# at-cg/PHI

Measured on AMD Instinct MI355X. Metric: read Gbases/s scored (49-hap MHC graph stand-in synMHC-49); reads resident in HBM, parsing and H2D excluded, higher is better.
Workload: dtype u64

## Files before the change

### phi_amd/build.py

```python
import os
import subprocess
import sys

ROOT = os.path.dirname(os.path.dirname(os.path.abspath(__file__)))
CSRC = os.path.join(ROOT, "phi_amd", "csrc")
HIPCC = os.environ.get("HIPCC", "/opt/rocm/bin/hipcc")
ARCH = "gfx950"

HIP_SOURCES = ["sketch.hip", "sketch_pooled.hip", "table.hip", "anchors.hip", "contexts.hip", "dp.hip", "dp_events.hip", "phi_abi.hip", "phi_solve.hip", "solve_dev.hip", "phi_comm.hip", "phi_ipc.hip", "reads_text.hip", "walk_text.hip", "edit.hip", "edit_path.hip", "inflate.hip", "gfa_text.hip"]
HIP_HEADERS = ["phi_dev.h", "phi_kernels.h", "phi_ctx.h", "sketch.hip", "sketch_phases.inc", "sketch_minima.inc", "sketch_rounds.inc", "edit_band.inc", os.path.join("..", "..", "include", "phi_amd.h")]


def _run(cmd, cwd=None):
    print("+", " ".join(cmd), flush=True)
    subprocess.check_call(cmd, cwd=cwd)


def _stale(target, deps):
    if not os.path.exists(target):
        return True
    t = os.path.getmtime(target)
    return any(os.path.getmtime(d) > t for d in deps if os.path.exists(d))


EXTRA_FLAGS = {"sketch_pooled.hip": ["-mllvm", "-disable-machine-licm"]}


def build_device(force=False):
    objdir = os.path.join(ROOT, "build", "obj")
    os.makedirs(objdir, exist_ok=True)
    hdrs = [os.path.join(CSRC, h) for h in HIP_HEADERS]
    objs = []
    for src in HIP_SOURCES:
        s = os.path.join(CSRC, src)
        o = os.path.join(objdir, src.replace(".hip", ".o"))
        if force or _stale(o, [s] + hdrs):
            _run([HIPCC, f"--offload-arch={ARCH}", "-O3", "-std=c++17", "-fPIC", "-Wall", "-Wno-unused-function"]
                 + EXTRA_FLAGS.get(src, []) + ["-c", s, "-o", o])
        objs.append(o)
    lib = os.path.join(ROOT, "phi_amd", "libphi_amd.so")
    if force or _stale(lib, objs):
        tmp = f"{lib}.{os.getpid()}.tmp"
        _run([HIPCC, f"--offload-arch={ARCH}", "-shared", "-fPIC", "-o", tmp] + objs + ["-ldl"])
        os.replace(tmp, lib)
    return lib


def build_host(force=False):
    hostdir = os.path.join(CSRC, "host")
    if not os.path.isdir(hostdir):
        return None
    _run(["make", "-C", hostdir] + (["-B"] if force else []))
    return os.path.join(ROOT, "phi_amd", "libphi_host.so")


def build_all(force=False):
    build_device(force)
    build_host(force)


if __name__ == "__main__":
    build_all(force="--force" in sys.argv)
```

### phi_amd/csrc/sketch.hip

```cpp
#include <hip/hip_runtime.h>
#include <type_traits>
#include <hip/hip_ext.h>
#include "phi_dev.h"
#include "phi_kernels.h"
#ifndef PHI_ABL
#define PHI_ABL 0
#endif

#define TPB PHI_TPB
#define Q 8

int64_t phi_sketch_num_blocks(int64_t n_bases);


static __device__ __forceinline__ void pack_ascii_word(int64_t wi, const uint8_t *__restrict__ bases, int64_t n,
                                                       uint64_t *__restrict__ words, int64_t n_words,
                                                       uint32_t *__restrict__ badbits,
                                                       unsigned long long *__restrict__ n_bad)
{
    if (wi >= n_words + 4) return;
    if (wi >= n_words) {
        if (wi < n_words + 2) words[wi] = 0;
        if (badbits) badbits[wi] = 0;
        return;
// ... 275 lines not shown
            else {
                const KRef prev = window_best_bytes(A.ascii, a - 1, k, w);
                emit = !(prev.pos == best.pos && prev.rc == best.rc) && khash_bytes<LONGK>(A.ascii, prev, k) != h;
            }
        }
        const unsigned long long bal = __ballot(emit);
        bool novel = false;
        if (emit) {
            const int rank = n_emit + __popcll(bal & ((1ull << lane) - 1));
            if (MODE == PHI_MODE_WRITE) {
                A.out_hash[out_base + rank] = h;
                A.out_pos[out_base + rank] = pos;
            } else if (MODE == PHI_MODE_PROBE) {
                novel = probe_table(A, h);
            }
        }
        if (MODE == PHI_MODE_PROBE) {
            const OverflowArgs O{A.ov_list, A.ov_count, A.ov_cap, A.err};
            n_nov += overflow_novel(O, novel, h, lane);
        }
        n_emit += __popcll(bal);
    }
    (void)chunk;
}


#define WCH PHI_WCH
#define SWW 32
#define SBW 16
#define SM(l) s_mp[(l) + ((l) >> 3)]

__host__ __device__ static inline int phi_wave_mp_u64(int w)
{
    const int M = WCH + w, P = (M + 63) / 64;
    const int slots = ((M - 1) / P + 1) * P;
    return ((slots + 8) * 9) / 8 + 8;
}
__host__ __device__ static inline int phi_wave_items(int w, int k) { return 1 + WCH + WCH / (w + k + 1) + 2; }
__host__ __device__ static inline int phi_wave_region_u64(int w, int k, bool pos)
{
    const int item_bytes = pos ? 4 : 2;
    return phi_wave_mp_u64(w) + SWW + 2 * SBW + ((phi_wave_items(w, k) + 4) * item_bytes + 7) / 8
#if PHI_ABL == 4
           + 256
#endif
        ;
}

__device__ __forceinline__ uint64_t min_u62(uint64_t a, uint64_t b)
{
    double r;
    asm("v_min_f64 %0, %1, %2" : "=v"(r) : "v"(__longlong_as_double((long long)a)), "v"(__longlong_as_double((long long)b)));
    return (uint64_t)__double_as_longlong(r);
}

__device__ __forceinline__ uint64_t wave_prev_u64(uint64_t v, uint64_t first, int lane)
{
    const uint32_t lo = (uint32_t)__builtin_amdgcn_update_dpp(0, (int)(uint32_t)v, 0x138, 0xF, 0xF, false);
    const uint32_t hi = (uint32_t)__builtin_amdgcn_update_dpp(0, (int)(uint32_t)(v >> 32), 0x138, 0xF, 0xF, false);
    const uint64_t p = ((uint64_t)hi << 32) | lo;
    return lane == 0 ? first : p;
}

__device__ __forceinline__ int wave_scan_inclusive(int v)
{
    v += __builtin_amdgcn_update_dpp(0, v, 0x111, 0xF, 0xF, true);
    v += __builtin_amdgcn_update_dpp(0, v, 0x112, 0xF, 0xF, true);
    v += __builtin_amdgcn_update_dpp(0, v, 0x114, 0xF, 0xF, true);
    v += __builtin_amdgcn_update_dpp(0, v, 0x118, 0xF, 0xF, true);
    v += __builtin_amdgcn_update_dpp(0, v, 0x142, 0xA, 0xF, false);
    v += __builtin_amdgcn_update_dpp(0, v, 0x143, 0xC, 0xF, false);
    return v;
}

template <int MODE>
static __device__ __forceinline__ void bytes_role(const PhiSketchArgs &A, const unsigned long long *batch_bad,
                                                  int64_t blk, int64_t n_blk, unsigned long long *s_all)
{
    const int lane = threadIdx.x & 63, wid = threadIdx.x >> 6;
    if (!A.allslow && batch_bad && *batch_bad == 0) return;
    const int64_t N = A.n_bases;
    const int64_t n_chunks = (N + WCH - 1) / WCH;
    const int64_t n_sw = N / 64 + 2;
    unsigned long long *s_bits = s_all + (size_t)wid * 2 * SBW, *s_bad = s_bits + SBW;
    for (int64_t chunk = blk * (TPB / 64) + wid; chunk < n_chunks; chunk += n_blk * (TPB / 64)) {
        const int64_t c0 = chunk * WCH;
        unsigned long long my_bad = 0;
        wave_sync();
        if (lane < SBW) {
            const int64_t wi = (c0 >> 6) - 1 + lane;
            s_bits[lane] = (wi >= 0 && wi < n_sw) ? A.starts[wi] : 0;
        } else if (lane < 2 * SBW) {
            const int64_t wi = (c0 >> 6) - 1 + (lane - SBW);
            if (A.badbits) my_bad = (wi >= 0 && wi < n_sw) ? A.badbits[wi] : 0;
            s_bad[lane - SBW] = my_bad;
        }
        const bool chunk_bad = __ballot(my_bad != 0) != 0ull;
        wave_sync();
        int n_emit = 0, n_nov = 0;
        if (A.allslow || chunk_bad) {
            const int64_t out_base = (MODE == PHI_MODE_WRITE) ? A.block_off[chunk] : 0;
            if (A.k > PHI_MAX_K_PACKED) slow_windows<MODE, true>(A, c0, chunk, lane, A.k, A.w, s_bits, s_bad, A.allslow != 0, out_base, n_emit, n_nov);
            else slow_windows<MODE>(A, c0, chunk, lane, A.k, A.w, s_bits, s_bad, A.allslow != 0, out_base, n_emit, n_nov);
        }
        if (MODE == PHI_MODE_COUNT) {
            if (lane == 0) A.block_cnt[chunk] = n_emit;
        }
    }
}



template <class AT>
__device__ __forceinline__ void clean_finish(const AT &A, int64_t gw, int64_t n_waves, int lane)
{
    if (gw == 0 && lane == 0 && A.ov_zero) *A.ov_zero = 0;
    if (A.ipc_mb && A.ipc_need) {
        while (__hip_atomic_load(A.ipc_mb + PHI_MB_GATHERED, __ATOMIC_RELAXED, __HIP_MEMORY_SCOPE_AGENT) < A.ipc_need) __builtin_amdgcn_s_sleep(32);
    }
    if (gw * 64 < A.q_n_hit_words)
        for (int64_t i = gw * 64 + lane; i < A.q_n_hit_words; i += n_waves * 64) A.q_hit_words[i] = 0;
    if (gw * 64 < A.q_n_stripe_words)
        for (int64_t i = gw * 64 + lane; i < A.q_n_stripe_words; i += n_waves * 64) A.q_stripes[i] = 0;
}

struct StartProbe { int64_t base; int64_t v; int64_t nx; };
__device__ __forceinline__ StartProbe start_probe_issue(const PhiSketchArgs &A, int64_t c0, int lane)
{
    const int64_t lo_b = c0 - 64 > 0 ? c0 - 64 : 0;
    int64_t g = (int64_t)(((unsigned long long)lo_b * A.reads_per_base_q32) >> 32) - 24;
    g = g < 0 ? 0 : (g > A.n_reads - 63 ? (A.n_reads - 63 > 0 ? A.n_reads - 63 : 0) : g);
    StartProbe p;
    p.base = g;
    const int64_t idx = g + lane;
    p.v = idx <= A.n_reads ? A.read_off[idx] : INT64_MAX;
    p.nx = idx + 1 <= A.n_reads ? A.read_off[idx + 1] : INT64_MAX;
    return p;
}
__device__ __forceinline__ void set_start_bit(unsigned long long *s_bits, int64_t p, int64_t lo_b)
{
    const int bit = (int)(p - lo_b);
    atomicOr(reinterpret_cast<unsigned int *>(s_bits) + (bit >> 5), 1u << (bit & 31));
}
__device__ __forceinline__ void start_bits_from_offsets(const PhiSketchArgs &A, int64_t c0, int lane, StartProbe pr,
                                                        unsigned long long *s_bits)
{
    const int64_t lo_b = c0 - 64, hi_b = lo_b + 64 * SBW;
    const unsigned long long ge = __ballot(pr.v >= lo_b), lt = __ballot(pr.v < hi_b);
    if ((pr.base == 0 || !(ge & 1ull)) && !(lt >> 63)) {
        if (pr.base + lane < A.n_reads && pr.v >= lo_b && pr.v < hi_b && pr.nx > pr.v) set_start_bit(s_bits, pr.v, lo_b);
        return;
    }
    {
        int64_t vm = __shfl(pr.v, 32, 64);
        if (vm == INT64_MAX) vm = A.n_bases;
        int64_t nb_all = A.n_bases, nr_all = A.n_reads;
        asm volatile("" : "+s"(nb_all), "+s"(nr_all));
        const double mean = (double)nb_all / (double)nr_all;
        int64_t g = pr.base + 32 + (int64_t)((double)(lo_b - vm) / mean) - 24;
        g = g < 0 ? 0 : (g > A.n_reads - 63 ? (A.n_reads - 63 > 0 ? A.n_reads - 63 : 0) : g);
        const int64_t idx = g + lane;
        const int64_t v2 = idx <= A.n_reads ? A.read_off[idx] : INT64_MAX;
        const int64_t nx2 = idx + 1 <= A.n_reads ? A.read_off[idx + 1] : INT64_MAX;
        const unsigned long long ge2 = __ballot(v2 >= lo_b), lt2 = __ballot(v2 < hi_b);
        if ((g == 0 || !(ge2 & 1ull)) && !(lt2 >> 63)) {
            if (idx < A.n_reads && v2 >= lo_b && v2 < hi_b && nx2 > v2) set_start_bit(s_bits, v2, lo_b);
            return;
        }
    }
    int64_t lo = 0, hi = A.n_reads;
    int64_t base = pr.base, stride = 1, v = pr.v;
    for (int round = 0; round < 64 && lo < hi; round++) {
        if (round) {
            stride = (hi - lo + 63) / 64;
            base = lo;
            const int64_t idx = base + lane * stride;
            v = idx <= A.n_reads ? A.read_off[idx] : INT64_MAX;
        }
        const unsigned long long g2 = __ballot(v >= lo_b);
        const int f = g2 ? __ffsll((long long)g2) - 1 : 64;
        if (f == 0) { hi = base < hi ? base : hi; }
        else {
            const int64_t below = base + (int64_t)(f - 1) * stride;
            lo = below + 1 > lo ? below + 1 : lo;
            if (f < 64) { const int64_t at = base + (int64_t)f * stride; hi = at < hi ? at : hi; }
        }
    }
    for (int64_t r = lo + lane;; r += 64) {
        int64_t p = INT64_MAX, nx = INT64_MAX;
        if (r < A.n_reads) { p = A.read_off[r]; nx = A.read_off[r + 1]; }
        if (p >= lo_b && p < hi_b && nx > p) set_start_bit(s_bits, p, lo_b);
        if (__shfl(p, 63, 64) >= hi_b) break;
    }
}

__device__ __forceinline__ void start_bits_uniform(const PhiSketchArgs &A, int64_t c0, int lane, unsigned long long *s_bits)
{
    const int64_t org = c0 - 64, hi_b = org + 64 * SBW;
    const int64_t from = org > 0 ? org : 0;
    const uint32_t L = (uint32_t)A.uniform_len;
    if (A.n_bases <= 0xFFFFFFFFll) {
        const uint32_t x = (uint32_t)__builtin_amdgcn_readfirstlane((int)(uint32_t)from);
        uint32_t q = __umulhi(x, A.inv_len_q32);
        uint32_t r = x - q * L;
        if (r >= L) { q++; r -= L; }
        const uint32_t first = x + (r ? L - r : 0u);
        const uint64_t p = (uint64_t)first + (uint64_t)(uint32_t)lane * (uint64_t)L;
        if (first >= x && (int64_t)p < hi_b && (int64_t)p < A.n_bases) set_start_bit(s_bits, (int64_t)p, org);
        return;
    }
    int64_t q = (int64_t)((double)from * A.inv_len);
    int64_t r = from - q * (int64_t)L;
    if (r < 0) { q--; r += L; }
    if (r >= (int64_t)L) { q++; r -= L; }
    const int64_t p = (q + (r != 0) + lane) * (int64_t)L;
    if (p < hi_b && p < A.n_bases) set_start_bit(s_bits, p, org);
}

template <int ONE = 0>
__device__ __forceinline__ uint4 load_bases16(const uint8_t *__restrict__ ascii, int64_t N, int64_t c0, int lane)
{
    const int64_t b = c0 - 32 + 16 * (int64_t)lane;
    if (b >= 0 && b + 16 <= N && (((uintptr_t)ascii + (uintptr_t)b) & 15) == 0) return *reinterpret_cast<const uint4 *>(ascii + b);
    uint32_t x[4] = {0x41414141u, 0x41414141u, 0x41414141u, 0x41414141u};
    if (b + 16 > 0 && b < N) {
#pragma unroll
        for (int j = 0; j < 16; j++)
            if (b + j >= 0 && b + j < N) x[j >> 2] = (x[j >> 2] & ~(0xFFu << (8 * (j & 3)))) | ((uint32_t)ascii[b + j] << (8 * (j & 3)));
    }
    return make_uint4(x[0], x[1], x[2], x[3]);
}

#ifndef PHI_SKETCH_POOLED_TU
template <int MODE, bool WIDE, int KT, int WT>
__global__ void __launch_bounds__(TPB, MODE == PHI_MODE_PROBE ? 6 : 1) phi_sketch_kernel(PhiSketchArgs A)
{
    constexpr bool FUSED = MODE == PHI_MODE_PROBE;
    constexpr bool NEED_POS = MODE == PHI_MODE_WRITE;
    constexpr bool FMIN = !NEED_POS && KT > 0 && KT <= 31;
    extern __shared__ uint64_t s_dyn[];

    const int lane = threadIdx.x & 63, wid = threadIdx.x >> 6;
    const int k = KT > 0 ? KT : A.k, w = WT ? WT : A.w;
    const int64_t N = A.n_bases;
    const int64_t chunk = (int64_t)blockIdx.x * (TPB / 64) + wid;
    const int64_t c0 = chunk * WCH;
    if (FUSED && A.ipc_mb && chunk == 0 && lane == 0)
        __hip_atomic_store(A.ipc_mb + PHI_MB_SCORED, A.ipc_scored, __ATOMIC_RELEASE, __HIP_MEMORY_SCOPE_AGENT);
    if (c0 >= N) {
        if (FUSED && A.q_clean) clean_finish(A, chunk, (int64_t)gridDim.x * (TPB / 64), lane);
        return;
    }
    const uint64_t kmask = phi_kmask(k);
    const int M = WCH + w;
    const int span = w + k - 1;
    const bool have_bad = FUSED || A.badbits != nullptr;

    using MetaT = typename std::conditional<NEED_POS, uint32_t, uint16_t>::type;
    constexpr uint32_t ITEM_FIRST = NEED_POS ? 1u << 31 : 1u << 15;
    constexpr uint32_t ITEM_NOEMIT = NEED_POS ? 1u << 30 : 1u << 14;
    uint64_t *s_mp = s_dyn + (size_t)wid * phi_wave_region_u64(w, k, NEED_POS);
    uint64_t *s_words = s_mp + phi_wave_mp_u64(w);
    unsigned long long *s_bits = (unsigned long long *)(s_words + SWW);
    unsigned long long *s_bad = s_bits + SBW;
    MetaT *s_meta = (MetaT *)(s_bad + SBW);
    uint64_t *s_q = s_mp + lane * (Q + 1);

    constexpr bool POOL = false;
    bool chunk_bad = false;
    int ncand = 0, n_emit = 0, n_log = 0, n_nov_slow = 0;
    int64_t out_base = 0;
    uint4 xn = make_uint4(0, 0, 0, 0);
    const int ci = 0, mine = 1;
    const int64_t stride = 0;
#include "sketch_phases.inc"

#if PHI_ABL == 15
    { asm volatile("" :: "v"(ncand)); return; }
#endif
#if PHI_ABL == 2
    ncand = 0;
#endif
#include "sketch_rounds.inc"

    if (FUSED && chunk_bad) {
        int n_emit_slow = 0;
        slow_windows<MODE>(A, c0, chunk, lane, k, w, s_bits, s_bad, false, 0, n_emit_slow, n_nov_slow);
        n_emit += n_emit_slow;
    }
    if (FUSED && A.q_clean) clean_finish(A, chunk, (int64_t)gridDim.x * (TPB / 64), lane);
    if (MODE == PHI_MODE_COUNT) {
        if (lane == 0) A.block_cnt[chunk] = n_emit;
    } else if (MODE == PHI_MODE_PROBE) {
        if (lane == 0) {
            const int cap = 1 << A.nov_shift;
            A.nov_cnt[A.log_base + chunk] = (uint16_t)(n_log < cap ? n_log : cap);
            const int n_nov_wave = n_log + n_nov_slow;
            const int stripe = (int)(chunk & (PHI_STRIPES - 1)) * 8;
            if (n_nov_wave && A.n_logged) atomicAdd(A.n_logged + stripe, (unsigned long long)n_nov_wave);
            if (n_emit && A.n_emitted) atomicAdd(A.n_emitted + stripe, (unsigned long long)n_emit);
        }
    }
}

__host__ __device__ static inline int phi_win_items_u64(int w, int k) { return ((phi_wave_items(w, k) + 4) * 2 + 7) / 8; }
__host__ __device__ static inline int phi_win_mp_u64(int R, int s, int w, int k)
{
    const int kmers = 9 * R * s;
    const int minima = 9 * (64 + 1) + phi_win_items_u64(w, k);
    return kmers > minima ? kmers : minima;
}
__host__ __device__ static inline int phi_win_region_u64(int R, int s, int w, int k) { return phi_win_mp_u64(R, s, w, k); }

__device__ __forceinline__ void stage_bad_bits(const uint8_t *__restrict__ ascii, int64_t N, int64_t c0, int lane,
                                               unsigned long long *s_bad)
{
    uint32_t bad = 0;
    if (lane < 62) {
        const uint4 v = load_bases16<1>(ascii, N, c0, lane);
        const uint32_t x[4] = {v.x, v.y, v.z, v.w};
#pragma unroll
        for (int b = 0; b < 16; b++) bad |= (uint32_t)(!phi_is_acgt((x[b >> 2] >> (8 * (b & 3))) & 0xFFu)) << b;
    }
    reinterpret_cast<uint16_t *>(s_bad)[lane < 62 ? lane + 2 : lane - 62] = (uint16_t)bad;
}

__device__ __forceinline__ void slow_windows_reads(const PhiSketchArgs &A, int64_t r0, int nr, int L, int V, int64_t c0, int lane,
                                                   int k, int w, const unsigned long long *s_bad, int &n_emit, int &n_nov)
{
    const int span = w + k - 1, n_win = nr * V;
    for (int q0 = 0; q0 < n_win; q0 += 64) {
        const int q = q0 + lane;
        const int rl = q / V, v = q - rl * V;
        const int64_t a = (r0 + rl) * (int64_t)L + v;
        const int lp = (int)(a - (c0 - 64));
        const bool todo = q < n_win && range_has_bit(s_bad, lp - 1, lp + span - 1);
        bool emit = false;
        uint64_t h = 0;
        if (todo) {
            const KRef best = window_best_bytes(A.ascii, a, k, w);
            h = khash_bytes<false>(A.ascii, best, k);
            if (v == 0) emit = h != PHI_EMPTY_KEY;
            else {
                const KRef prev = window_best_bytes(A.ascii, a - 1, k, w);
                emit = !(prev.pos == best.pos && prev.rc == best.rc) && khash_bytes<false>(A.ascii, prev, k) != h;
            }
        }
        const unsigned long long bal = __ballot(emit);
        const bool novel = emit && probe_table(A, h);
        const OverflowArgs O{A.ov_list, A.ov_count, A.ov_cap, A.err};
        n_nov += overflow_novel(O, novel, h, lane);
        n_emit += __popcll(bal);
    }
}

template <bool WIDE, int KT, int WT>
__global__ void __launch_bounds__(TPB, 7) phi_sketch_win_kernel(PhiSketchArgs A)
{
    constexpr int MODE = PHI_MODE_PROBE;
    constexpr bool NEED_POS = false;
    constexpr bool FMIN = KT > 0 && KT <= 31;
    static_assert(KT >= 0, "k <= 32");
    extern __shared__ uint64_t s_dyn[];

    const int lane = threadIdx.x & 63, wid = threadIdx.x >> 6;
    const int k = KT > 0 ? KT : A.k, w = WT ? WT : A.w;
    const int64_t N = A.n_bases;
    const int L = A.uniform_len, span = w + k - 1, V = L - span + 1;
    const int G = (V + Q - 1) / Q, s = G + (w + Q - 1) / Q, R = A.win_reads;
    const int64_t chunk = (int64_t)blockIdx.x * (TPB / 64) + wid;
    const int64_t rd0 = chunk * R;
    if (A.ipc_mb && chunk == 0 && lane == 0)
        __hip_atomic_store(A.ipc_mb + PHI_MB_SCORED, A.ipc_scored, __ATOMIC_RELEASE, __HIP_MEMORY_SCOPE_AGENT);
    if (rd0 >= A.n_reads) {
        if (A.q_clean) clean_finish(A, chunk, (int64_t)gridDim.x * (TPB / 64), lane);
        return;
    }
    const int nr = A.n_reads - rd0 < R ? (int)(A.n_reads - rd0) : R;
    const uint64_t kmask = phi_kmask(k);
    const int64_t c0 = (rd0 * (int64_t)L) & ~(int64_t)31;
    const int rl = (int)(((float)lane + 0.5f) * (1.0f / (float)G)), j = lane - rl * G;
    const bool live = rl < nr;

    using MetaT = uint16_t;
    constexpr uint32_t ITEM_FIRST = 1u << 15;
    constexpr uint32_t ITEM_NOEMIT = 1u << 14;
    uint64_t *s_mp = s_dyn + (size_t)wid * phi_win_region_u64(R, s, w, k);
    uint64_t *s_words = s_mp;
    unsigned long long *s_bad = (unsigned long long *)s_mp;
    MetaT *s_meta = (MetaT *)(s_mp + 9 * (64 + 1));
    uint64_t *s_q = s_mp + (live ? 9 * (rl * s + j) : 0);

    bool chunk_bad;
    {
        const uint4 v = load_bases16<1>(A.ascii, N, c0, lane);
        const uint32_t x[4] = {v.x, v.y, v.z, v.w};
        uint32_t code = 0, bad = 0;
#pragma unroll
        for (int q = 0; q < 4; q++) {
            const uint32_t t = ((x[q] >> 1) ^ (x[q] >> 2)) & 0x03030303u;
            const uint32_t c8 = (t * 0x40100401u) >> 24;
            code = (code << 8) | c8;
            if (__builtin_amdgcn_perm(0x54474341u, 0x54474341u, t) != (x[q] & 0xDFDFDFDFu)) {
#pragma unroll
                for (int b = 0; b < 4; b++) bad |= (uint32_t)(!phi_is_acgt((x[q] >> (8 * b)) & 0xFFu)) << (4 * q + b);
            }
        }
        reinterpret_cast<uint32_t *>(s_words)[lane ^ 1] = code;
        chunk_bad = __ballot(lane < 62 && bad != 0) != 0ull;
    }
    wave_sync();

    {
        int n = 0, u = 0;
        uint64_t F = 0, Rc = 0, nxt = 0;
        if (live) {
            const int n_km = L - k + 1, P = (n_km + G - 1) / G;
            const int t0 = j * P;
            n = n_km - t0 < P ? n_km - t0 : P;
            if (n > 0) {
                const int lb = (int)((rd0 + rl) * (int64_t)L + t0 - c0) + 32;
                F = lds_extract64(s_words, lb) >> (64 - 2 * k);
                nxt = lds_extract64(s_words, lb + k);
                u = 8 * s * rl + 1 + t0;
            }
        }
        wave_sync();
        if (n > 0) {
            Rc = phi_revcomp(F, k);
            for (int i = 0; i < n; i++, u++) {
                if (i) {
                    const uint64_t b = nxt >> 62;
                    nxt <<= 2;
                    F = ((F << 2) | b) & kmask;
                    Rc = (Rc >> 2) | ((3 - b) << (2 * k - 2));
                }
                s_mp[u + (u >> 3)] = FMIN ? min_u62(F, Rc) : (F < Rc ? F : Rc);
            }
        }
    }
    wave_sync();

#include "sketch_minima.inc"

    if (chunk_bad) {
        wave_sync();
        stage_bad_bits(A.ascii, N, c0, lane, s_bad);
        wave_sync();
    }
    uint32_t cflag = 0, fflag = 0, pflag = 0;
    if (live) {
        const int imax = V - Q * j < Q ? V - Q * j : Q;
        const uint32_t in_read = (2u << imax) - 2u;
        const uint32_t first = j == 0 ? 2u : 0u;
        uint32_t changed = 0;
#pragma unroll
        for (int i = 1; i <= Q; i++) changed |= (uint32_t)(wv[i] != wv[i - 1]) << i;
        uint32_t dall = 0, reseed = 0;
        if (chunk_bad) {
            const int lp0 = (int)((rd0 + rl) * (int64_t)L + Q * j - 1 - (c0 - 64));
            for (int i = 0; i <= Q; i++) dall |= (uint32_t)range_has_bit(s_bad, lp0 + i - 1, lp0 + i + span - 1) << i;
            reseed = ~dall & (dall << 1);
        }
        cflag = in_read & ~dall & (first | changed | reseed);
        fflag = cflag & first;
        pflag = cflag & reseed & ~first;
    }
    int ncand, coff;
    {
        const int cnt = __popc(cflag) + __popc(pflag);
        const int v = wave_scan_inclusive(cnt);
        ncand = __builtin_amdgcn_readlane(v, 63);
        coff = v - cnt;
    }
    wave_sync();
    {
        uint64_t *s_w = s_mp + 9 * lane;
#define SW(x) s_w[(x) + ((x) >> 3)]
        if (lane == 0) SW(0) = wv[0];
#pragma unroll
        for (int i = 1; i <= Q; i++) SW(i) = wv[i];
#undef SW
        int c = coff + 1;
        if (!chunk_bad) {
            for (uint32_t f = cflag; f; f &= f - 1) {
                const uint32_t i = (uint32_t)__ffs((int)f) - 1;
                s_meta[c++] = (MetaT)((uint32_t)(lane * Q) + i + (((fflag >> i) & 1u) ? ITEM_FIRST : 0u));
            }
        } else {
#pragma unroll
            for (int i = 1; i <= Q; i++) {
                if ((cflag >> i) & 1u) {
                    if ((pflag >> i) & 1u) s_meta[c++] = (MetaT)((uint32_t)(lane * Q + i - 1) | ITEM_NOEMIT);
                    s_meta[c++] = (MetaT)((uint32_t)(lane * Q + i) | (((fflag >> i) & 1u) ? ITEM_FIRST : 0u));
                }
            }
        }
        if (coff == 0 && cflag) s_meta[0] = (MetaT)((uint32_t)(lane * Q + __ffs((int)cflag) - 2) | ITEM_NOEMIT);
    }
    wave_sync();
#undef SQ

    int n_emit = 0, n_log = 0, n_nov_slow = 0;
    const int64_t out_base = 0;
#include "sketch_rounds.inc"

    if (chunk_bad) {
        unsigned long long *s_bad_s = (unsigned long long *)(s_dyn + (size_t)__builtin_amdgcn_readfirstlane(wid) * phi_win_region_u64(R, s, w, k));
        wave_sync();
        stage_bad_bits(A.ascii, N, c0, lane, s_bad_s);
        wave_sync();
        int n_emit_slow = 0;
        slow_windows_reads(A, rd0, nr, L, V, c0, lane, k, w, s_bad_s, n_emit_slow, n_nov_slow);
        n_emit += n_emit_slow;
    }
    {
        const KArgs P = kargs_now();
        if (P->q_clean) clean_finish(*P, chunk, (int64_t)gridDim.x * (TPB / 64), lane);
        if (lane == 0) {
            const int cap = 1 << P->nov_shift;
            P->nov_cnt[P->log_base + chunk] = (uint16_t)(n_log < cap ? n_log : cap);
            const int n_nov_wave = n_log + n_nov_slow;
            const int stripe = (int)(chunk & (PHI_STRIPES - 1)) * 8;
            if (n_nov_wave && P->n_logged) atomicAdd(P->n_logged + stripe, (unsigned long long)n_nov_wave);
            if (n_emit && P->n_emitted) atomicAdd(P->n_emitted + stripe, (unsigned long long)n_emit);
        }
    }
}

#else
template <bool WIDE, int KT, int WT>
__global__ void __launch_bounds__(TPB, 6) phi_sketch_pool_kernel(PhiSketchArgs A)
{
    constexpr int MODE = PHI_MODE_PROBE;
    constexpr bool FUSED = true, NEED_POS = false, POOL = true;
    constexpr bool FMIN = KT > 0 && KT <= 31;
    static_assert(KT >= 0, "k <= 32");
    extern __shared__ uint64_t s_dyn[];

    const int k = KT > 0 ? KT : A.k, w = WT ? WT : A.w;
    const int64_t N = A.n_bases;
    const int64_t n_chunks_all = (N + WCH - 1) / WCH;
    const int64_t stride = (int64_t)A.wave_stride;
    int mine;
    {
        const int lane = threadIdx.x & 63, wid = threadIdx.x >> 6;
        const int64_t gw = (int64_t)blockIdx.x * (TPB / 64) + wid;
        if (A.ipc_mb && gw == 0 && lane == 0)
            __hip_atomic_store(A.ipc_mb + PHI_MB_SCORED, A.ipc_scored, __ATOMIC_RELEASE, __HIP_MEMORY_SCOPE_AGENT);
        if (gw >= n_chunks_all || gw >= stride) {
            if (A.q_clean) clean_finish(A, gw, (int64_t)gridDim.x * (TPB / 64), lane);
            return;
        }
        mine = __builtin_amdgcn_readfirstlane((int)((n_chunks_all - gw + stride - 1) / stride));
    }
    const uint64_t kmask = phi_kmask(k);
    const int M = WCH + w;
    const int span = w + k - 1;
    const bool have_bad = true;

    using MetaT = uint16_t;
    constexpr uint32_t ITEM_FIRST = 1u << 15;
    constexpr uint32_t ITEM_NOEMIT = 1u << 14;
    int n_emit = 0, n_log = 0, n_nov_slow = 0;
    uint64_t pv = 0;
    uint32_t pf = 0;
    int pend = 0;
    uint64_t carry = PHI_EMPTY_KEY;

    uint4 xn = load_bases16(A.ascii, N, ((int64_t)blockIdx.x * (TPB / 64) + (threadIdx.x >> 6)) * WCH, (int)(threadIdx.x & 63));
    for (int ci = 0; ci <= mine; ci++) {
    uint32_t tid = threadIdx.x;
    asm volatile("" : "+v"(tid));
    const int lane = (int)(tid & 63u), wid = __builtin_amdgcn_readfirstlane((int)(tid >> 6));
    const int64_t gw = (int64_t)blockIdx.x * (TPB / 64) + wid;
    const int64_t chunk = gw + ci * stride;
    const int64_t c0 = chunk * WCH;
    int ncand = 0;
    bool chunk_bad = false;
    int64_t out_base = 0;
    (void)out_base;
    uint64_t *s_mp = s_dyn + (size_t)wid * phi_wave_region_u64(w, k, NEED_POS);
    uint64_t *s_words = s_mp + phi_wave_mp_u64(w);
    unsigned long long *s_bits = (unsigned long long *)(s_words + SWW);
    unsigned long long *s_bad = s_bits + SBW;
    MetaT *s_meta = (MetaT *)(s_bad + SBW);
    uint64_t *s_q = s_mp + lane * (Q + 1);
    if (ci) wave_sync();
    if (ci < mine) {
#include "sketch_phases.inc"

#if PHI_ABL == 15
    { asm volatile("" :: "v"(ncand)); return; }
#endif
#if PHI_ABL == 2
    ncand = 0;
#endif
    }
    {
        const int n_items = ncand > 0 ? ncand + 1 : 0;
        const bool flush = ci == mine;
        int taken = 0;
        while (pend + (n_items - taken) >= 64 || (flush && pend > 0)) {
            uint64_t v = pv;
            uint32_t f = pf;
            if (lane >= pend && !flush) {
                const uint32_t meta = s_meta[taken + lane - pend];
                v = SM((int)(meta & 0x3FFu));
                f = meta >> 14;
                if (FMIN) v |= (uint64_t)f << 62;
            }
            const bool valid = !flush || lane < pend;
            taken += 64 - pend;
            pend = 0;
            const uint64_t h = phi_kmer_hash(FMIN ? (v & 0x3FFFFFFFFFFFFFFFull) : v, k);
            const uint32_t flg = FMIN ? (uint32_t)(v >> 62) : f;
            const uint64_t hp = wave_prev_u64(h, carry, lane);
            carry = ((uint64_t)(uint32_t)__builtin_amdgcn_readlane((int)(uint32_t)(h >> 32), 63) << 32) |
                    (uint32_t)__builtin_amdgcn_readlane((int)(uint32_t)h, 63);
            const bool emit = valid && !(flg & 1u) && ((flg & 2u) || h != hp);
            const unsigned long long bal = __ballot(emit);
            bool novel = false;
            const KArgs R = kargs_now();
#if PHI_ABL == 5
            asm volatile("" :: "v"(h));
#else
            if (emit) {
                const ProbeArgs P{R->u_rt, R->u_bmask, R->hit, R->err};
                novel = probe_table(P, h);
            }
#endif
            const unsigned long long ib = __ballot(novel);
            const int pos = n_log + __popcll(ib & ((1ull << lane) - 1));
            const int sh = R->nov_shift, room = mine << sh;
            if (novel && pos < room) R->nov_log[((R->log_base + gw + (int64_t)(pos >> sh) * stride) << sh) + (pos & ((1 << sh) - 1))] = h;
            n_log += __popcll(ib);
            if (n_log > room) {
                const OverflowArgs O{R->ov_list, R->ov_count, R->ov_cap, R->err};
                overflow_novel(O, novel && pos >= room, h, lane);
            }
            n_emit += __popcll(bal);
        }
        const int rem = flush ? 0 : n_items - taken;
        if (lane >= pend && lane < pend + rem) {
            const uint32_t meta = s_meta[taken + lane - pend];
            pv = SM((int)(meta & 0x3FFu));
            pf = meta >> 14;
            if (FMIN) pv |= (uint64_t)pf << 62;
        }
        pend += rem;
    }

    if (chunk_bad) {
        int n_emit_slow = 0;
        slow_windows<MODE>(A, c0, chunk, lane, k, w, s_bits, s_bad, false, 0, n_emit_slow, n_nov_slow);
        n_emit += n_emit_slow;
    }
    }
    uint32_t tid_end = threadIdx.x;
    asm volatile("" : "+v"(tid_end));
    const int lane = (int)(tid_end & 63u);
    const int64_t gw = (int64_t)blockIdx.x * (TPB / 64) + __builtin_amdgcn_readfirstlane((int)(tid_end >> 6));
    {
        const KArgs R = kargs_now();
        if (R->q_clean) clean_finish(*R, gw, (int64_t)gridDim.x * (TPB / 64), lane);
        {
            const int sh = R->nov_shift, cap = 1 << sh;
            for (int j = lane; j < mine; j += 64) {
                const int left = n_log - (j << sh);
                R->nov_cnt[R->log_base + gw + j * stride] = (uint16_t)(left < 0 ? 0 : left < cap ? left : cap);
            }
        }
        const int n_nov_wave = n_log + n_nov_slow;
        if (lane == 0) {
            const int stripe = (int)(gw & (PHI_STRIPES - 1)) * 8;
            if (n_nov_wave && R->n_logged) atomicAdd(R->n_logged + stripe, (unsigned long long)n_nov_wave);
            if (n_emit && R->n_emitted) atomicAdd(R->n_emitted + stripe, (unsigned long long)n_emit);
        }
    }
}

#endif

#ifdef PHI_SKETCH_POOLED_TU
void phi_launch_sketch_pooled(hipStream_t st, unsigned nb, size_t lds, const PhiSketchArgs &A, hipEvent_t t0, hipEvent_t t1)
{
    if (A.k == 31 && A.w == 25) hipExtLaunchKernelGGL((phi_sketch_pool_kernel<true, 31, 25>), dim3(nb), dim3(TPB), lds, st, t0, t1, 0, A);
    else if (A.w > Q) hipExtLaunchKernelGGL((phi_sketch_pool_kernel<true, 0, 0>), dim3(nb), dim3(TPB), lds, st, t0, t1, 0, A);
    else hipExtLaunchKernelGGL((phi_sketch_pool_kernel<false, 0, 0>), dim3(nb), dim3(TPB), lds, st, t0, t1, 0, A);
}
#else
void phi_launch_sketch_pooled(hipStream_t st, unsigned nb, size_t lds, const PhiSketchArgs &A, hipEvent_t t0, hipEvent_t t1);

template <int MODE>
__global__ void __launch_bounds__(TPB) phi_sketch_bytes_kernel(PhiSketchArgs A, const unsigned long long *batch_bad)
{
    __shared__ unsigned long long s_all[(TPB / 64) * 2 * SBW];
    bytes_role<MODE>(A, batch_bad, blockIdx.x, gridDim.x, s_all);
}

__global__ void __launch_bounds__(1024) phi_scan_counts_kernel(const int32_t *__restrict__ cnt, int64_t n,
                                                               int64_t *__restrict__ off)
{
    __shared__ int64_t s_w[16];
    __shared__ int64_t s_carry;
    const int tid = threadIdx.x, lane = tid & 63, wid = tid >> 6;
    if (tid == 0) s_carry = 0;
    __syncthreads();
    for (int64_t base = 0; base < n; base += 4096) {
        const int64_t i0 = base + 4 * (int64_t)tid;
        int32_t v[4];
#pragma unroll
        for (int j = 0; j < 4; j++) v[j] = i0 + j < n ? cnt[i0 + j] : 0;
        const int64_t c = (int64_t)v[0] + v[1] + v[2] + v[3];
        int64_t inc = c;
#pragma unroll
        for (int d = 1; d < 64; d <<= 1) {
            const int64_t t = __shfl_up(inc, d, 64);
            if (lane >= d) inc += t;
        }
        if (lane == 63) s_w[wid] = inc;
        const int64_t carry = s_carry;
        __syncthreads();
        int64_t run = carry + inc - c;
        for (int x = 0; x < wid; x++) run += s_w[x];
#pragma unroll
        for (int j = 0; j < 4; j++) {
            if (i0 + j < n) off[i0 + j] = run;
            run += v[j];
        }
        if (tid == 1023) s_carry = run;
        __syncthreads();
    }
    if (tid == 0) off[n] = s_carry;
}


void phi_launch_pack_ascii(hipStream_t st, const uint8_t *bases, int64_t n, uint64_t *words, int64_t n_words,
                           uint32_t *badbits, unsigned long long *n_bad)
{
    if (n_words <= 0) return;
    const int64_t nb = (n_words + 4 + 255) / 256;
    hipLaunchKernelGGL(phi_pack_ascii_kernel, dim3((unsigned)nb), dim3(256), 0, st, bases, n, words, n_words, badbits,
                       n_bad);
}

void phi_launch_mark_starts(hipStream_t st, const int64_t *seq_off, int64_t n_seq, unsigned long long *starts)
{
    if (n_seq <= 0) return;
    const int64_t nb = (n_seq + 255) / 256;
    hipLaunchKernelGGL(phi_mark_starts_kernel, dim3((unsigned)nb), dim3(256), 0, st, seq_off, n_seq, starts);
}

void phi_launch_sketch_bytes(hipStream_t st, int mode, const PhiSketchArgs &A, const unsigned long long *batch_bad)
{
    const int64_t nchunks = phi_sketch_num_blocks(A.n_bases);
    if (nchunks <= 0) return;
    int64_t nb = (nchunks + TPB / 64 - 1) / (TPB / 64);
    if (!A.allslow && nb > 1024) nb = 1024;
    if (mode == PHI_MODE_COUNT)
        hipLaunchKernelGGL(phi_sketch_bytes_kernel<PHI_MODE_COUNT>, dim3((unsigned)nb), dim3(TPB), 0, st, A, batch_bad);
    else
        hipLaunchKernelGGL(phi_sketch_bytes_kernel<PHI_MODE_WRITE>, dim3((unsigned)nb), dim3(TPB), 0, st, A, batch_bad);
}

void phi_launch_reset_reads(hipStream_t st, uint64_t *hit_words, int64_t n_hit_words, uint64_t *stripes, int64_t n_stripe_words)
{
    int64_t n = n_hit_words > n_stripe_words ? n_hit_words : n_stripe_words;
    int64_t nb = (n + 255) / 256;
    if (nb > 2048) nb = 2048;
    if (nb < 1) nb = 1;
    hipLaunchKernelGGL(phi_reset_reads_kernel, dim3((unsigned)nb), dim3(256), 0, st, hit_words, n_hit_words, stripes, n_stripe_words);
}

int64_t phi_sketch_num_blocks(int64_t n_bases) { return n_bases <= 0 ? 0 : (n_bases + WCH - 1) / WCH; }

template <int MODE>
static void launch_sketch_mode(hipStream_t st, unsigned nb, size_t lds, const PhiSketchArgs &A, hipEvent_t t0, hipEvent_t t1, bool pooled)
{
    if constexpr (MODE == PHI_MODE_PROBE) {
        if (pooled) { phi_launch_sketch_pooled(st, nb, lds, A, t0, t1); return; }
    }
    if constexpr (MODE != PHI_MODE_WRITE) {
        if (A.k == 31 && A.w == 25) {
            hipExtLaunchKernelGGL((phi_sketch_kernel<MODE, true, 31, 25>), dim3(nb), dim3(TPB), lds, st, t0, t1, 0, A);
            return;
        }
    }
    if constexpr (MODE == PHI_MODE_PROBE) {
        if (A.k > PHI_MAX_K_PACKED) {
            hipExtLaunchKernelGGL((phi_sketch_kernel<MODE, true, -1, 0>), dim3(nb), dim3(TPB), lds, st, t0, t1, 0, A);
            return;
        }
    }
    if (A.w > Q) hipExtLaunchKernelGGL((phi_sketch_kernel<MODE, true, 0, 0>), dim3(nb), dim3(TPB), lds, st, t0, t1, 0, A);
    else hipExtLaunchKernelGGL((phi_sketch_kernel<MODE, false, 0, 0>), dim3(nb), dim3(TPB), lds, st, t0, t1, 0, A);
}

static int64_t pool_min_chunks()
{
    int64_t min_chunks = 4 * 6144;
    if (const char *e = getenv("PHI_SKETCH_POOL_MIN")) min_chunks = atoll(e);
    return min_chunks;
}

int phi_sketch_win_reads(int k, int w, int64_t uniform_len, int64_t n_reads, int64_t n_bases)
{
    if (uniform_len <= 0 || n_reads <= 0 || k > PHI_MAX_K_PACKED) return 0;
    int force = -1;
    if (const char *e = getenv("PHI_SKETCH_WINDOWS")) force = atoi(e) ? 1 : 0;
    if (force == 0) return 0;
    const int64_t L = uniform_len, V = L - (k + w - 1) + 1;
    if (V < 1 || L > 928) return 0;
    const int G = (int)((V + Q - 1) / Q), s = G + (w + Q - 1) / Q;
    if (G > 64 || (L - k + 1 + G - 1) / G > 32) return 0;
    int R = 64 / G;
    if (R > 928 / L) R = (int)(928 / L);
    while (R > 0 && phi_win_region_u64(R, s, w, k) + SWW + SBW > phi_wave_region_u64(w, k, false)) R--;
    if (R < 1) return 0;
    if (force != 1 && (R * L < WCH + WCH / 8 || (getenv("PHI_SKETCH_POOL_MIN") && phi_sketch_num_blocks(n_bases) >= pool_min_chunks()))) return 0;
    return R;
}

int64_t phi_sketch_read_chunks(int k, int w, int64_t uniform_len, int64_t n_reads, int64_t n_bases)
{
    const int R = phi_sketch_win_reads(k, w, uniform_len, n_reads, n_bases);
    return R > 0 ? (n_reads + R - 1) / R : phi_sketch_num_blocks(n_bases);
}

void phi_launch_sketch(hipStream_t st, int mode, const PhiSketchArgs &A0, hipEvent_t t0, hipEvent_t t1)
{
    const int64_t nchunks = phi_sketch_num_blocks(A0.n_bases);
    if (nchunks <= 0) return;
    PhiSketchArgs A = A0;
    if (mode == PHI_MODE_PROBE) {
        const int R = phi_sketch_win_reads(A.k, A.w, A.uniform_len, A.n_reads, A.n_bases);
        if (R > 0) {
            A.win_reads = R;
            const int64_t waves = (A.n_reads + R - 1) / R;
            const unsigned nb = (unsigned)((waves + TPB / 64 - 1) / (TPB / 64));
            const int V = (int)(A.uniform_len - (A.k + A.w - 1) + 1);
            const int s = (V + Q - 1) / Q + (A.w + Q - 1) / Q;
            const size_t lds = (size_t)phi_win_region_u64(R, s, A.w, A.k) * 8 * (TPB / 64);
            if (A.k == 31 && A.w == 25) hipExtLaunchKernelGGL((phi_sketch_win_kernel<true, 31, 25>), dim3(nb), dim3(TPB), lds, st, t0, t1, 0, A);
            else if (A.w > Q) hipExtLaunchKernelGGL((phi_sketch_win_kernel<true, 0, 0>), dim3(nb), dim3(TPB), lds, st, t0, t1, 0, A);
            else hipExtLaunchKernelGGL((phi_sketch_win_kernel<false, 0, 0>), dim3(nb), dim3(TPB), lds, st, t0, t1, 0, A);
            return;
        }
    }
    int64_t njobs = nchunks;
    bool pooled = false;
    if (mode == PHI_MODE_PROBE && A.k <= PHI_MAX_K_PACKED) {
        int64_t slots = 4 * 256 * 4 * 6;
        const int64_t min_chunks = pool_min_chunks();
        if (const char *e = getenv("PHI_SKETCH_WAVES")) slots = atoll(e) > 0 ? atoll(e) : slots;
        if (nchunks >= min_chunks) {
            int64_t m = (nchunks + slots - 1) / slots;
            if (m < 3) m = 3;
            njobs = (nchunks + m - 1) / m;
            if (njobs > 0x7FFFFFFF) njobs = 0x7FFFFFFF;
            A.wave_stride = (int32_t)njobs;
            pooled = true;
        }
    }
    const unsigned nb = (unsigned)((njobs + TPB / 64 - 1) / (TPB / 64));
    const size_t lds = (size_t)phi_wave_region_u64(A.w, A.k, mode == PHI_MODE_WRITE) * 8 * (TPB / 64);
    if (mode == PHI_MODE_COUNT) launch_sketch_mode<PHI_MODE_COUNT>(st, nb, lds, A, t0, t1, false);
    else if (mode == PHI_MODE_WRITE) launch_sketch_mode<PHI_MODE_WRITE>(st, nb, lds, A, t0, t1, false);
    else launch_sketch_mode<PHI_MODE_PROBE>(st, nb, lds, A, t0, t1, pooled);
}

void phi_launch_scan_counts(hipStream_t st, const int32_t *cnt, int64_t n, int64_t *off)
{
    hipLaunchKernelGGL(phi_scan_counts_kernel, dim3(1), dim3(1024), 0, st, cnt, n, off);
}

__global__ void phi_warm_sketch_kernel() {}
void phi_warm_sketch(hipStream_t st) { hipLaunchKernelGGL(phi_warm_sketch_kernel, dim3(1), dim3(64), 0, st); }
#endif
```

Measured before the change: 429.7.

## Add compile-time specialized window sketch kernel for k=31 w=25 150bp reads

Adds a separate translation unit with a window-sketch kernel fully specialized on k=31, w=25 and read length 150 (five reads per wave). It builds 31-mer canonical values directly from a packed 2-bit code array with alignbit extracts and a bit-reverse complement, instead of going through the generic per-lane k-mer path. It also writes them into LDS with fixed offsets and a fast path for clean chunks. The launcher dispatches to it when the parameters match, and an env var can disable it. This adds code size and a narrow fast path that only applies to this read length and k/w pair.

```diff
diff --git a/phi_amd/build.py b/phi_amd/build.py
--- a/phi_amd/build.py
+++ b/phi_amd/build.py
@@ -7,7 +7,7 @@
 HIPCC = os.environ.get("HIPCC", "/opt/rocm/bin/hipcc")
 ARCH = "gfx950"
 
-HIP_SOURCES = ["sketch.hip", "sketch_pooled.hip", "table.hip", "anchors.hip", "contexts.hip", "dp.hip", "dp_events.hip", "phi_abi.hip", "phi_solve.hip", "solve_dev.hip", "phi_comm.hip", "phi_ipc.hip", "reads_text.hip", "walk_text.hip", "edit.hip", "edit_path.hip", "inflate.hip", "gfa_text.hip"]
+HIP_SOURCES = ["sketch.hip", "sketch_pooled.hip", "sketch_win_fixed.hip", "table.hip", "anchors.hip", "contexts.hip", "dp.hip", "dp_events.hip", "phi_abi.hip", "phi_solve.hip", "solve_dev.hip", "phi_comm.hip", "phi_ipc.hip", "reads_text.hip", "walk_text.hip", "edit.hip", "edit_path.hip", "inflate.hip", "gfa_text.hip"]
 HIP_HEADERS = ["phi_dev.h", "phi_kernels.h", "phi_ctx.h", "sketch.hip", "sketch_phases.inc", "sketch_minima.inc", "sketch_rounds.inc", "edit_band.inc", os.path.join("..", "..", "include", "phi_amd.h")]
 
 
diff --git a/phi_amd/csrc/sketch.hip b/phi_amd/csrc/sketch.hip
--- a/phi_amd/csrc/sketch.hip
+++ b/phi_amd/csrc/sketch.hip
@@ -601,6 +601,7 @@
         }
     }
 }
+#endif
 
 __host__ __device__ static inline int phi_win_items_u64(int w, int k) { return ((phi_wave_items(w, k) + 4) * 2 + 7) / 8; }
 __host__ __device__ static inline int phi_win_mp_u64(int R, int s, int w, int k)
@@ -653,6 +654,7 @@
     }
 }
 
+#ifndef PHI_SKETCH_POOLED_TU
 template <bool WIDE, int KT, int WT>
 __global__ void __launch_bounds__(TPB, 7) phi_sketch_win_kernel(PhiSketchArgs A)
 {
@@ -827,7 +829,7 @@
     }
 }
 
-#else
+#elif !defined(PHI_SKETCH_WIN_FIXED_TU)
 template <bool WIDE, int KT, int WT>
 __global__ void __launch_bounds__(TPB, 6) phi_sketch_pool_kernel(PhiSketchArgs A)
 {
@@ -981,7 +983,8 @@
 
 #endif
 
-#ifdef PHI_SKETCH_POOLED_TU
+#ifdef PHI_SKETCH_WIN_FIXED_TU
+#elif defined(PHI_SKETCH_POOLED_TU)
 void phi_launch_sketch_pooled(hipStream_t st, unsigned nb, size_t lds, const PhiSketchArgs &A, hipEvent_t t0, hipEvent_t t1)
 {
     if (A.k == 31 && A.w == 25) hipExtLaunchKernelGGL((phi_sketch_pool_kernel<true, 31, 25>), dim3(nb), dim3(TPB), lds, st, t0, t1, 0, A);
@@ -990,6 +993,7 @@
 }
 #else
 void phi_launch_sketch_pooled(hipStream_t st, unsigned nb, size_t lds, const PhiSketchArgs &A, hipEvent_t t0, hipEvent_t t1);
+bool phi_launch_sketch_win_fixed(hipStream_t st, unsigned nb, size_t lds, const PhiSketchArgs &A, hipEvent_t t0, hipEvent_t t1);
 
 template <int MODE>
 __global__ void __launch_bounds__(TPB) phi_sketch_bytes_kernel(PhiSketchArgs A, const unsigned long long *batch_bad)
@@ -1141,6 +1145,7 @@
             const int V = (int)(A.uniform_len - (A.k + A.w - 1) + 1);
             const int s = (V + Q - 1) / Q + (A.w + Q - 1) / Q;
             const size_t lds = (size_t)phi_win_region_u64(R, s, A.w, A.k) * 8 * (TPB / 64);
+            if (phi_launch_sketch_win_fixed(st, nb, lds, A, t0, t1)) return;
             if (A.k == 31 && A.w == 25) hipExtLaunchKernelGGL((phi_sketch_win_kernel<true, 31, 25>), dim3(nb), dim3(TPB), lds, st, t0, t1, 0, A);
             else if (A.w > Q) hipExtLaunchKernelGGL((phi_sketch_win_kernel<true, 0, 0>), dim3(nb), dim3(TPB), lds, st, t0, t1, 0, A);
             else hipExtLaunchKernelGGL((phi_sketch_win_kernel<false, 0, 0>), dim3(nb), dim3(TPB), lds, st, t0, t1, 0, A);
diff --git a/phi_amd/csrc/sketch_win_fixed.hip b/phi_amd/csrc/sketch_win_fixed.hip
--- /dev/null
+++ b/phi_amd/csrc/sketch_win_fixed.hip
@@ -0,0 +1,203 @@
+#define PHI_SKETCH_POOLED_TU 1
+#define PHI_SKETCH_WIN_FIXED_TU 1
+#include "sketch.hip"
+
+__device__ __forceinline__ uint32_t revcomp16(uint32_t x)
+{
+    x = __builtin_bitreverse32(x);
+    return ~(((x >> 1) & 0x55555555u) | ((x << 1) & 0xAAAAAAAAu));
+}
+
+template <int S>
+__device__ __forceinline__ uint64_t bits62(uint32_t u0, uint32_t u1, uint32_t u2)
+{
+    static_assert(S >= 0 && S <= 34, "inside the 96 bits");
+    uint32_t lo, hi;
+    if constexpr (S >= 32) {
+        lo = __builtin_amdgcn_alignbit(u0, u1, S - 32);
+        hi = (u0 >> (S - 32)) & 0x3FFFFFFFu;
+    } else {
+        lo = __builtin_amdgcn_alignbit(u1, u2, S);
+        hi = __builtin_amdgcn_alignbit(u0, u1, S) & 0x3FFFFFFFu;
+    }
+    return ((uint64_t)hi << 32) | lo;
+}
+
+template <int KT, int WT, int LT>
+__global__ void __launch_bounds__(TPB, 7) phi_sketch_winfix_kernel(PhiSketchArgs A)
+{
+    constexpr int MODE = PHI_MODE_PROBE;
+    constexpr bool NEED_POS = false, WIDE = true, FMIN = true;
+    constexpr int k = KT, w = WT, L = LT, span = w + k - 1, V = L - span + 1;
+    constexpr int G = (V + Q - 1) / Q, s = G + (w + Q - 1) / Q, R = 64 / G;
+    constexpr int NKM = L - k + 1, P = NKM / G;
+    static_assert(k == 31 && w > Q, "31-mers: values below 2^62, two 62-bit extracts of 48 bases");
+    static_assert(V == Q * G && NKM == P * G && P == 10, "every window and k-mer of a lane exists; the store offsets below");
+    static_assert(R * L <= 928 && R * G <= 64, "the staging of phase 0");
+    extern __shared__ uint64_t s_dyn[];
+
+    const int lane = threadIdx.x & 63, wid = threadIdx.x >> 6;
+    const int64_t chunk = (int64_t)blockIdx.x * (TPB / 64) + wid;
+    const int64_t rd0 = chunk * R;
+    const int64_t c0 = (rd0 * L) & ~(int64_t)31;
+    const int64_t N = A.n_bases;
+    const uint4 bv = load_bases16<1>(A.ascii, N, c0, lane);
+    if (A.ipc_mb && chunk == 0 && lane == 0)
+        __hip_atomic_store(A.ipc_mb + PHI_MB_SCORED, A.ipc_scored, __ATOMIC_RELEASE, __HIP_MEMORY_SCOPE_AGENT);
+    if (rd0 >= A.n_reads) {
+        if (A.q_clean) clean_finish(A, chunk, (int64_t)gridDim.x * (TPB / 64), lane);
+        return;
+    }
+    const int nr = A.n_reads - rd0 < R ? (int)(A.n_reads - rd0) : R;
+    const int rl = (int)((unsigned)lane / (unsigned)G), j = lane - rl * G;
+    const bool live = rl < nr;
+
+    using MetaT = uint16_t;
+    constexpr uint32_t ITEM_FIRST = 1u << 15;
+    constexpr uint32_t ITEM_NOEMIT = 1u << 14;
+    uint64_t *s_mp = s_dyn + (size_t)wid * phi_win_region_u64(R, s, w, k);
+    uint32_t *s_code = (uint32_t *)s_mp;
+    unsigned long long *s_bad = (unsigned long long *)s_mp;
+    MetaT *s_meta = (MetaT *)(s_mp + 9 * (64 + 1));
+    uint64_t *s_q = s_mp + (live ? 9 * (rl * s + j) : 0);
+
+    bool chunk_bad;
+    {
+        const uint32_t x[4] = {bv.x, bv.y, bv.z, bv.w};
+        uint32_t code = 0, bad = 0;
+#pragma unroll
+        for (int q = 0; q < 4; q++) {
+            const uint32_t t = ((x[q] >> 1) ^ (x[q] >> 2)) & 0x03030303u;
+            const uint32_t c8 = (t * 0x40100401u) >> 24;
+            code = (code << 8) | c8;
+            if (__builtin_amdgcn_perm(0x54474341u, 0x54474341u, t) != (x[q] & 0xDFDFDFDFu)) {
+#pragma unroll
+                for (int b = 0; b < 4; b++) bad |= (uint32_t)(!phi_is_acgt((x[q] >> (8 * b)) & 0xFFu)) << (4 * q + b);
+            }
+        }
+        s_code[lane] = code;
+        chunk_bad = __ballot(lane < 62 && bad != 0) != 0ull;
+    }
+    wave_sync();
+
+    {
+        const int lb = (int)((rd0 * L) & 31) + rl * L + P * j + 32;
+        const int d0 = (lb - 1) >> 4, rsh = 30 - 2 * ((lb - 1) & 15);
+        const uint32_t d[4] = {s_code[d0], s_code[d0 + 1], s_code[d0 + 2], s_code[d0 + 3]};
+        wave_sync();
+        const uint32_t u0 = __builtin_amdgcn_alignbit(d[0], d[1], rsh);
+        const uint32_t u1 = __builtin_amdgcn_alignbit(d[1], d[2], rsh);
+        const uint32_t u2 = __builtin_amdgcn_alignbit(d[2], d[3], rsh);
+        const uint32_t z0 = revcomp16(u2), z1 = revcomp16(u1), z2 = revcomp16(u0);
+        uint64_t km[P];
+#define KM(i) km[i] = min_u62(bits62<34 - 2 * (i)>(u0, u1, u2), bits62<2 * (i)>(z0, z1, z2))
+        KM(0); KM(1); KM(2); KM(3); KM(4); KM(5); KM(6); KM(7); KM(8); KM(9);
+#undef KM
+        if (live) {
+            const int u = 8 * s * rl + 1 + P * j, m = j & 3;
+            uint64_t *b0 = s_mp + u + (u >> 3);
+            uint64_t *b1 = b0 + (m == 3), *b2 = b0 + (m >= 2), *b3 = b0 + (m >= 1);
+            b0[0] = km[0];
+            b1[1] = km[1]; b1[2] = km[2];
+            b2[3] = km[3]; b2[4] = km[4];
+            b3[5] = km[5]; b3[6] = km[6];
+            b0[8] = km[7]; b0[9] = km[8];
+            b1[10] = km[9];
+        }
+    }
+    wave_sync();
+
+#include "sketch_minima.inc"
+
+    if (chunk_bad) {
+        wave_sync();
+        stage_bad_bits(A.ascii, N, c0, lane, s_bad);
+        wave_sync();
+    }
+    uint32_t cflag = 0, fflag = 0, pflag = 0;
+    if (live) {
+        constexpr uint32_t in_read = (2u << Q) - 2u;
+        const uint32_t first = j == 0 ? 2u : 0u;
+        uint32_t changed = 0;
+#pragma unroll
+        for (int i = 1; i <= Q; i++) changed |= (uint32_t)(wv[i] != wv[i - 1]) << i;
+        uint32_t dall = 0, reseed = 0;
+        if (chunk_bad) {
+            const int lp0 = (int)((rd0 * L) & 31) + rl * L + Q * j - 1 + 64;
+            for (int i = 0; i <= Q; i++) dall |= (uint32_t)range_has_bit(s_bad, lp0 + i - 1, lp0 + i + span - 1) << i;
+            reseed = ~dall & (dall << 1);
+        }
+        cflag = in_read & ~dall & (first | changed | reseed);
+        fflag = cflag & first;
+        pflag = cflag & reseed & ~first;
+    }
+    int ncand, coff;
+    {
+        const int cnt = __popc(cflag) + __popc(pflag);
+        const int v = wave_scan_inclusive(cnt);
+        ncand = __builtin_amdgcn_readlane(v, 63);
+        coff = v - cnt;
+    }
+    wave_sync();
+    {
+        uint64_t *s_w = s_mp + 9 * lane;
+#define SW(x) s_w[(x) + ((x) >> 3)]
+        if (lane == 0) SW(0) = wv[0];
+#pragma unroll
+        for (int i = 1; i <= Q; i++) SW(i) = wv[i];
+#undef SW
+        int c = coff + 1;
+        if (!chunk_bad) {
+            for (uint32_t f = cflag; f; f &= f - 1) {
+                const uint32_t i = (uint32_t)__ffs((int)f) - 1;
+                s_meta[c++] = (MetaT)((uint32_t)(lane * Q) + i + (((fflag >> i) & 1u) ? ITEM_FIRST : 0u));
+            }
+        } else {
+#pragma unroll
+            for (int i = 1; i <= Q; i++) {
+                if ((cflag >> i) & 1u) {
+                    if ((pflag >> i) & 1u) s_meta[c++] = (MetaT)((uint32_t)(lane * Q + i - 1) | ITEM_NOEMIT);
+                    s_meta[c++] = (MetaT)((uint32_t)(lane * Q + i) | (((fflag >> i) & 1u) ? ITEM_FIRST : 0u));
+                }
+            }
+        }
+        if (coff == 0 && cflag) s_meta[0] = (MetaT)((uint32_t)(lane * Q + __ffs((int)cflag) - 2) | ITEM_NOEMIT);
+    }
+    wave_sync();
+#undef SQ
+
+    int n_emit = 0, n_log = 0, n_nov_slow = 0;
+    const int64_t out_base = 0;
+#include "sketch_rounds.inc"
+
+    if (chunk_bad) {
+        unsigned long long *s_bad_s = (unsigned long long *)(s_dyn + (size_t)__builtin_amdgcn_readfirstlane(wid) * phi_win_region_u64(R, s, w, k));
+        wave_sync();
+        stage_bad_bits(A.ascii, N, c0, lane, s_bad_s);
+        wave_sync();
+        int n_emit_slow = 0;
+        slow_windows_reads(A, rd0, nr, L, V, c0, lane, k, w, s_bad_s, n_emit_slow, n_nov_slow);
+        n_emit += n_emit_slow;
+    }
+    {
+        const KArgs PA = kargs_now();
+        if (PA->q_clean) clean_finish(*PA, chunk, (int64_t)gridDim.x * (TPB / 64), lane);
+        if (lane == 0) {
+            const int cap = 1 << PA->nov_shift;
+            PA->nov_cnt[PA->log_base + chunk] = (uint16_t)(n_log < cap ? n_log : cap);
+            const int n_nov_wave = n_log + n_nov_slow;
+            const int stripe = (int)(chunk & (PHI_STRIPES - 1)) * 8;
+            if (n_nov_wave && PA->n_logged) atomicAdd(PA->n_logged + stripe, (unsigned long long)n_nov_wave);
+            if (n_emit && PA->n_emitted) atomicAdd(PA->n_emitted + stripe, (unsigned long long)n_emit);
+        }
+    }
+}
+
+bool phi_launch_sketch_win_fixed(hipStream_t st, unsigned nb, size_t lds, const PhiSketchArgs &A, hipEvent_t t0, hipEvent_t t1)
+{
+    if (!(A.k == 31 && A.w == 25 && A.uniform_len == 150 && A.win_reads == 5)) return false;
+    if (const char *e = getenv("PHI_SKETCH_WIN_FIXED"))
+        if (!atoi(e)) return false;
+    hipExtLaunchKernelGGL((phi_sketch_winfix_kernel<31, 25, 150>), dim3(nb), dim3(TPB), lds, st, t0, t1, 0, A);
+    return true;
+}
```

Result: faster. 452.6, median of 6 (+5.3%).
